# zijinxuxu/PDFNet

Hardware: AMD Instinct MI355X
Metric: train-step images/sec @256x256 RGB-D B=32 (higher is better)
Workload: dtype f32

## Files before the change

include/pdfnet_hip.h:

```cpp
#ifndef PDFNET_HIP_H
#define PDFNET_HIP_H
#ifdef __cplusplus
extern "C" {
#endif

#define PDF_E_BADARG (-1)
#define PDF_E_WORKSPACE (-2)
#define PDF_ACT_NONE 0
#define PDF_ACT_RELU 1
#define PDF_ACT_LRELU01 2


int pdf_linear_fwd(const float* x, const float* w, const float* bias, float* y,
                   int M, int N, int K, int ldx, int ldw, int ldy, int act, void* stream);
int pdf_linear_bwd_weight(const float* x, const float* dy, float* dw, float* db, float* ws, long ws_floats,
                          int M, int N, int K, int ldx, int lddy, int accumulate, void* stream);
long pdf_wgrad_workspace_floats(int M, int NI, int NJ);
int pdf_init(void);
int pdf_debug_init_device(void);
int pdf_debug_kernel_timing(int on);
int pdf_set_stats_output(float* part, long cap_floats);
long pdf_stats_result_tiles(void);
long pdf_stats_result_rows(void);
int pdf_set_bn_tile_stats(const float* part, long tiles, long rows_per_tile);
// ... 230 lines not shown
int pdf_mano_split_coeff_bwd(const float* params, float* dparams, int ldp, long HW, const long* ind, const float* K, int B, int input_res, int down,
                             const float* dorient, const float* dpose, const float* dtrans, void* stream);


typedef struct PdfCallOpts {
    const void* op0_bf16; const void* op1_bf16;
    void* out_bf16;
    const void* bn_x_bf16;
    float* stats_out; long stats_cap;
    long stats_tiles; long stats_rows;
    const float* tile_stats; long tile_n; long tile_rows;
    const float* in_scale; const float* in_shift;
    const void* op1_bf16_t;
    float* ws; long ws_floats;
    const float* wino_v;
} PdfCallOpts;
long pdf_conv2d_winograd_v_offset(int N, int H, int W, int Cin, int Cout, int KH, int KW, int stride, int pad);
int pdf_linear_fwd_x(const float* x, const float* w, const float* bias, float* y, int M, int N, int K, int ldx, int ldw, int ldy, int act, void* stream, PdfCallOpts* opts);
int pdf_linear_fwd_pair_x(const float* x, const float* w0, const float* w1, const float* b0, const float* b1, float* y, int M, int N, int K, int ldx, int ldw, int ldy, int act, void* stream, PdfCallOpts* opts);
int pdf_linear_bwd_data_x(const float* dy, const float* w, float* dx, int M, int N, int K, int lddy, int ldw, int lddx, void* stream, PdfCallOpts* opts);
int pdf_linear_bwd_data_pair_x(const float* dy, const float* w0, const float* w1, float* dx, int M, int N, int K, int lddy, int ldw, int lddx, void* stream, PdfCallOpts* opts);
int pdf_conv2d_fwd_x(const float* x, const float* w, const float* bias, float* y, int N, int H, int W, int Cin, int ldx, int Cout, int KH, int KW, int stride, int pad, int OH, int OW, int ldy, int act, void* stream, PdfCallOpts* opts);
int pdf_conv2d_bwd_data_x(const float* dy, const float* w, float* dx, int N, int H, int W, int Cin, int lddx, int Cout, int KH, int KW, int stride, int pad, int OH, int OW, int lddy, void* stream, PdfCallOpts* opts);
int pdf_conv2d_bwd_data_add_x(const float* dy, const float* w, float* dx, int N, int H, int W, int Cin, int lddx, int Cout, int KH, int KW, int stride, int pad, int OH, int OW, int lddy, void* stream, PdfCallOpts* opts);
int pdf_linear_bwd_weight_x(const float* x, const float* dy, float* dw, float* db, float* ws, long ws_floats, int M, int N, int K, int ldx, int lddy, int accumulate, void* stream, PdfCallOpts* opts);
int pdf_linear_bwd_weight_pair_x(const float* x, const float* dy, float* dw0, float* dw1, float* db0, float* db1, float* ws, long ws_floats, int M, int N, int K, int ldx, int lddy, int accumulate, void* stream, PdfCallOpts* opts);
int pdf_conv2d_bwd_weight_x(const float* x, const float* dy, float* dw, float* db, float* ws, long ws_floats, int N, int H, int W, int Cin, int ldx, int Cout, int KH, int KW, int stride, int pad, int OH, int OW, int lddy, int accumulate, void* stream, PdfCallOpts* opts);
int pdf_deconv2d_fwd_x(const float* x, const float* w, const float* bias, float* y, int N, int H, int W, int Cin, int ldx, int Cout, int KH, int KW, int stride, int pad, int OH, int OW, int ldy, void* stream, PdfCallOpts* opts);
int pdf_deconv2d_bwd_data_x(const float* dy, const float* w, float* dx, int N, int H, int W, int Cin, int lddx, int Cout, int KH, int KW, int stride, int pad, int OH, int OW, int lddy, void* stream, PdfCallOpts* opts);
int pdf_deconv2d_bwd_weight_x(const float* x, const float* dy, float* dw, float* ws, long ws_floats, int N, int H, int W, int Cin, int ldx, int Cout, int KH, int KW, int stride, int pad, int OH, int OW, int lddy, int accumulate, void* stream, PdfCallOpts* opts);
int pdf_bn_train_fwd_x(const float* x, int ldx, int C, long R, const float* gamma, const float* beta, float* running_mean, float* running_var, float momentum, float eps, const float* res, int ldr, int relu, float* y, int ldy, float* save_mean, float* save_rstd, float* scale, float* shift, float* ws, void* stream, PdfCallOpts* opts);
int pdf_bn_train_bwd_x(const float* dy, int lddy, const float* y, int ldy, int relu, const float* x, int ldx, const float* save_mean, const float* save_rstd, const float* gamma, const float* scale, const float* shift, int C, long R, float* dx, int lddx, float* dres, int lddr, float* dgamma, float* dbeta, int accumulate, float* ws, void* stream, PdfCallOpts* opts);
int pdf_bn_relu_maxk_fwd_x(const float* y, int ldy, int C, long R, int K, const float* gamma, const float* beta, float* running_mean, float* running_var, float momentum, float eps, int training, float* out, int ldo, int* arg, float* save_mean, float* save_rstd, float* scale, float* shift, float* ws, void* stream, PdfCallOpts* opts);
int pdf_l2norm_cat_fwd_x(int nparts, const float* const* x, const int* C, const float* const* w, float eps, long R, float* y, int ldy, float* const* norm, void* stream, PdfCallOpts* opts);
long pdf_conv2d_winograd_workspace_floats(int N, int H, int W, int Cin, int Cout, int KH, int KW, int stride, int pad, int backward);
int pdf_debug_armed_slots(void);
int pdf_debug_callopts_size(void);

int pdf_x3_split(const float* x, void* out, long n, long cs, void* stream);
long pdf_deconv2d_x3_workspace_floats(int N, int H, int W, int Cin, int Cout, int KH, int KW, int stride, int pad, int backward);
int pdf_set_x3_mode(int mode);
int pdf_stream_create(void** out, int priority, int* lo, int* hi);
int pdf_debug_x3_mode(void);
int pdf_debug_x3_stamps(unsigned long long* out);
int pdf_x3_batched_gemm_nt(const void* A3, long csA, const void* B3, long csB, float* C, int batch, long gsA, long gsB, long gsC, int M, int N, int K, int variant, int nprod, void* stream);
int pdf_batched_gemm_nt(const float* A, const float* B, float* C, int batch, long gsA, long gsB, long gsC, int M, int N, int K, void* stream);
int pdf_x3_batched_gemm_tn(const void* P3, long csP, const void* Q3, long csQ, float* slab, int batch, long gsP, long gsQ, int M, int NI, int NJ, int splits, int variant, int nprod, void* stream);
int pdf_batched_gemm_tn(const float* P, const float* Q, float* slab, int batch, long gsP, long gsQ, int M, int NI, int NJ, int splits, void* stream);

typedef struct PdfMeshLin { const float* w[2]; const float* b[2]; } PdfMeshLin;
typedef struct PdfMeshLN { const float* g[2]; const float* b[2]; } PdfMeshLN;
typedef struct PdfMeshGcn { PdfMeshLin fc1, fc2, sc; PdfMeshLN n2, n3; unsigned long long seed; } PdfMeshGcn;
typedef struct PdfMeshAttn {
    PdfMeshLN ln; PdfMeshLin q, k, v, fc; PdfMeshLN ffln; PdfMeshLin f1, f2;
    unsigned long long seed_att, seed_z, seed_t, seed_x;
// ... 55 lines not shown
```

pdfnet_amd/csrc/gemm.hip:

```cpp
#include "common.h"

#include "gemm_common.h"
#include "gemm_internal.h"

PDF_API long pdf_conv2d_winograd_v_offset(int N, int H, int W, int Cin, int Cout, int KH, int KW, int stride, int pad) {
    if (!pdf_internal_wino_eligible(N, H, W, Cin, Cout, KH, KW, stride, pad, 0) || !pdf_internal_wino_wgrad_eligible(N, H, W, Cin, Cout, KH, KW, stride, pad)) return -1;
    return pdf_internal_wino_v_offset(N, H, W, Cin, Cout);
}
PDF_API long pdf_conv2d_winograd_workspace_floats(int N, int H, int W, int Cin, int Cout, int KH, int KW, int stride, int pad, int backward) {
    if (backward == 2) return pdf_internal_wino_wgrad_eligible(N, H, W, Cin, Cout, KH, KW, stride, pad) ? pdf_internal_wino_wgrad_workspace(N, H, W, Cin, Cout) : 0;
    const int Ck = backward ? Cout : Cin, Cn = backward ? Cin : Cout;
    return pdf_internal_wino_eligible(N, H, W, Ck, Cn, KH, KW, stride, pad, backward) ? pdf_internal_wino_workspace(N, H, W, Ck, Cn, backward) : 0;
}

constexpr int WG_ISSUE_AT = 1;
typedef unsigned int u32x4v __attribute__((ext_vector_type(4)));
__device__ __forceinline__ float4 as_f4(const u32x4v& v) { return *reinterpret_cast<const float4*>(&v); }

template <int BM, int BN, int WM, int WN, bool FAST, bool KN, int BKT, bool BUF, bool AFF>
__device__ __forceinline__ void igemm_nt_body(const IGemm& g) {
    constexpr int NT = WM * WN * 64;
    constexpr int BK = BKT, LD = BK + 1;
    constexpr int TM = BM / WM / 32, TN = BN / WN / 32;
    constexpr int TPR = BK / 4, RPP = NT / TPR;
// ... 1319 lines not shown
}

int pdf_internal_batched_gemm(const float* A, const float* B, float* C, int batch, long gsA, long gsB, long gsC, int M, int N, int K, hipStream_t s) {
    IGemm g = {};
    g.A = A; g.B = B; g.C = C; g.bias = nullptr;
    g.M = M; g.N = N; g.K = K; g.Cin = K; g.lda = K; g.ldb = K; g.ldc = N;
    g.T = 1; g.plain_in = 1; g.plain_out = 1; g.act = 0;
    g.H = 1; g.W = M; g.QH = 1; g.QW = M; g.sy = 1; g.sx = 1;
    g.batch = batch; g.gsA = gsA; g.gsB = gsB; g.gsC = gsC;
    if (g_gemm_bf16) return PDF_E_BADARG;
    return launch_igemm(g, s, batch);
}

PDF_API long pdf_deconv2d_x3_workspace_floats(int N, int H, int W, int Cin, int Cout, int KH, int KW, int stride, int pad, int backward) {
    return g_gemm_bf16 ? 0 : pdf_internal_x3_deconv_workspace(N, H, W, Cin, Cout, KH, KW, stride, pad, backward);
}
static void conv_taps(IGemm& g, int KH, int KW, int pad, int dil) {
    g.T = KH * KW;
    for (int ky = 0; ky < KH; ++ky)
        for (int kx = 0; kx < KW; ++kx) {
            int t = ky * KW + kx;
            g.dy[t] = (int)(ky * dil - pad); g.dx[t] = (int)(kx * dil - pad); g.wt[t] = t;
        }
}

static IGemm linear_desc(const float* x, const float* w, const float* bias, float* y,
                         int M, int N, int K, int ldx, int ldw, int ldy, int act) {
    IGemm g = {};
    g.A = x; g.B = w; g.C = y; g.bias = bias;
    g.M = M; g.N = N; g.K = K; g.Cin = K; g.lda = ldx; g.ldb = ldw; g.ldc = ldy;
// ... 820 lines not shown
PDF_API int pdf_deconv2d_bwd_data(const float* dy, const float* w, float* dx,
                                  int N, int H, int W, int Cin, int lddx, int Cout, int KH, int KW,
                                  int stride, int pad, int OH, int OW, int lddy, void* stream) {
    return pdf_call_plain(pdf_deconv2d_bwd_data_impl, dy, w, dx, N, H, W, Cin, lddx, Cout, KH, KW, stride, pad, OH, OW, lddy, stream);
}


static int pdf_deconv2d_bwd_weight_impl(const float* x, const float* dy, float* dw, float* ws, long ws_floats,
                                    int N, int H, int W, int Cin, int ldx, int Cout, int KH, int KW,
                                    int stride, int pad, int OH, int OW, int lddy, int accumulate, void* stream, PdfCallOpts& co) {
    hipStream_t s = (hipStream_t)stream;
    if (KH * KW > MAX_TAPS) return PDF_E_BADARG;
    if (!g_gemm_bf16 && co.ws != nullptr && ldx == Cin && lddy == Cout) {
        const long need = pdf_internal_x3_deconv_workspace(N, H, W, Cin, Cout, KH, KW, stride, pad, 2);
        if (need > 0 && co.ws_floats >= need && ((uintptr_t)co.ws & 15) == 0) {
            if (KH != stride || pad != 0) return pdf_internal_x3_deconv_general_bwd_weight(x, dy, dw, co.ws, N, H, W, Cin, Cout, KH, stride, pad, OH, OW, lddy, accumulate, s);
            return pdf_internal_x3_deconv_bwd_weight(x, dy, dw, co.ws, N, H, W, Cin, Cout, KH, KW, stride, OH, OW, lddy, accumulate, s);
        }
    }
    WGemm g = {};
    g.P = x; g.Q = dy; g.P16 = co.op0_bf16; g.Q16 = co.op1_bf16; g.M = N * H * W; g.NI = Cin; g.Cq = Cout; g.T = KH * KW;
    g.ldp = ldx; g.ldq = lddy; g.ldw = KH * KW * Cout;
    g.H = OH; g.W = OW; g.QH = H; g.QW = W; g.sy = stride; g.sx = stride; g.plain_q = 0;
    for (int ky = 0; ky < KH; ++ky)
        for (int kx = 0; kx < KW; ++kx) {
            int t = ky * KW + kx;
            g.dy[t] = (int)(ky - pad); g.dx[t] = (int)(kx - pad); g.wt[t] = t;
        }
    return launch_wgemm(g, dw, ws, ws_floats, accumulate, s);
}
PDF_API int pdf_deconv2d_bwd_weight_x(const float* x, const float* dy, float* dw, float* ws, long ws_floats,
                                    int N, int H, int W, int Cin, int ldx, int Cout, int KH, int KW,
                                    int stride, int pad, int OH, int OW, int lddy, int accumulate, void* stream, PdfCallOpts* opts) {
    return pdf_call_x(opts, pdf_deconv2d_bwd_weight_impl, x, dy, dw, ws, ws_floats, N, H, W, Cin, ldx, Cout, KH, KW, stride, pad, OH, OW, lddy,
// ... 10 lines not shown
```

pdfnet_amd/csrc/gemm_internal.h:

```cpp
#pragma once
#include "common.h"

int pdf_internal_batched_gemm(const float* A, const float* B, float* C, int batch, long gsA, long gsB, long gsC, int M, int N, int K, hipStream_t s);
int pdf_internal_batched_wgemm(const float* P, const float* Q, float* slab, int batch, long gsP, long gsQ, int M, int NI, int NJ, int splits, hipStream_t s);

long pdf_internal_wino_workspace(int N, int H, int W, int Ck, int Cn, int flip);
int pdf_internal_wino_eligible(int N, int H, int W, int Ck, int Cn, int KH, int KW, int stride, int pad, int flip);
int pdf_internal_conv3x3_winograd(const float* x, int ldx, const float* w, const float* bias, float* y, int ldy, float* ws,
                                  int N, int H, int W, int Ck, int Cn, int act, int accum, int flip, const float* v_shared, hipStream_t s);
int pdf_internal_wino_wgrad_eligible(int N, int H, int W, int Cin, int Cout, int KH, int KW, int stride, int pad);
long pdf_internal_wino_wgrad_workspace(int N, int H, int W, int Cin, int Cout);
long pdf_internal_wino_v_offset(int N, int H, int W, int Ck, int Cn);
int pdf_internal_conv3x3_winograd_wgrad(const float* x, int ldx, const float* dy, int lddy, float* dw, float* db, float* ws,
                                        int N, int H, int W, int Cin, int Cout, int accumulate, const float* v_cached, hipStream_t s);

int pdf_internal_x3_mode();
int pdf_internal_x3_batched_gemm(const void* A3, long csA, const void* B3, long csB, float* C, int batch, long gsA, long gsB, long gsC,
                                 int M, int N, int K, int variant, int nprod, hipStream_t s);
int pdf_internal_x3_batched_wgemm(const void* P3, long csP, const void* Q3, long csQ, float* slab, int batch, long gsP, long gsQ,
                                  int M, int NI, int NJ, int splits, int variant, int nprod, hipStream_t s);
long pdf_internal_x3_deconv_workspace(int N, int H, int W, int Cin, int Cout, int KH, int KW, int stride, int pad, int backward);
int pdf_internal_x3_deconv_fwd(const float* x, const float* w, const float* bias, float* y, float* ws, int N, int H, int W, int Cin, int Cout,
                               int KH, int KW, int stride, int OH, int OW, int ldy, hipStream_t s);
int pdf_internal_x3_deconv_bwd_data(const float* dy, const float* w, float* dx, float* ws, int N, int H, int W, int Cin, int lddx, int Cout,
                                    int KH, int KW, int stride, int OH, int OW, int lddy, hipStream_t s);
int pdf_internal_x3_deconv_general_fwd(const float* x, const float* w, const float* bias, float* y, float* ws, int N, int H, int W, int Cin, int Cout,
                                       int K, int stride, int pad, int OH, int OW, int ldy, hipStream_t s);
int pdf_internal_x3_deconv_general_bwd_data(const float* dy, const float* w, float* dx, float* ws, int N, int H, int W, int Cin, int lddx, int Cout,
                                            int K, int stride, int pad, int OH, int OW, int lddy, hipStream_t s);
int pdf_internal_x3_deconv_general_bwd_weight(const float* x, const float* dy, float* dw, float* ws, int N, int H, int W, int Cin, int Cout,
                                              int K, int stride, int pad, int OH, int OW, int lddy, int accumulate, hipStream_t s);
int pdf_internal_x3_deconv_bwd_weight(const float* x, const float* dy, float* dw, float* ws, int N, int H, int W, int Cin, int Cout,
                                      int KH, int KW, int stride, int OH, int OW, int lddy, int accumulate, hipStream_t s);
```

pdfnet_amd/csrc/gemm_x3.hip:

```cpp
#include "gemm_common.h"
#include "gemm_internal.h"
#include <cstdio>

typedef __bf16 bf16x8v __attribute__((ext_vector_type(8)));
typedef short s16x4v __attribute__((ext_vector_type(4)));
typedef short s16x8v __attribute__((ext_vector_type(8)));
typedef int i32x4 __attribute__((ext_vector_type(4)));

__device__ __forceinline__ i32x4 x3_rsrc(const void* p, unsigned bytes) {
    const unsigned long long a = (unsigned long long)p;
    i32x4 r = {(int)(unsigned)(a & 0xffffffffu), (int)(unsigned)((a >> 32) & 0xffffu), (int)bytes, 0x00020000};
    return r;
}
__device__ __forceinline__ void x3_dma16(const i32x4& rsrc, unsigned lds_addr, unsigned voff) {
    asm volatile("s_mov_b32 m0, %0\n\tbuffer_load_dwordx4 %1, %2, 0 offen lds" ::"s"(lds_addr), "v"(voff), "s"(rsrc) : "memory");
}

__global__ __launch_bounds__(256) void x3_split_kernel(const float* __restrict__ x, unsigned short* __restrict__ o, long n8, long cs) {
    for (long i = blockIdx.x * 256L + threadIdx.x; i < n8; i += (long)gridDim.x * 256) {
        const float4 u = reinterpret_cast<const float4*>(x)[2 * i], v = reinterpret_cast<const float4*>(x)[2 * i + 1];
        uint4 h, m, l;
        pdf_x3_split2(u.x, u.y, h.x, m.x, l.x); pdf_x3_split2(u.z, u.w, h.y, m.y, l.y);
        pdf_x3_split2(v.x, v.y, h.z, m.z, l.z); pdf_x3_split2(v.z, v.w, h.w, m.w, l.w);
        *reinterpret_cast<uint4*>(o + 8 * i) = h;
// ... 679 lines not shown
PDF_API int pdf_set_x3_mode(int mode) { g_x3_mode = mode < 0 ? -1 : (mode & 7); return 0; }
PDF_API int pdf_debug_x3_mode(void) { return pdf_internal_x3_mode(); }
static int x3_deconv_mode() { return (pdf_internal_x3_mode() & 2) != 0; }
static long x3_ld(long K) { return K + 64; }
static long x3_deconv_general_workspace(int N, int H, int W, int Cin, int Cout, int K, int stride, int pad, int backward);
long pdf_internal_x3_deconv_workspace(int N, int H, int W, int Cin, int Cout, int KH, int KW, int stride, int pad, int backward) {
    if (!x3_deconv_mode() || KH != KW || stride < 2) return 0;
    if (KH != stride || pad != 0) return x3_deconv_general_workspace(N, H, W, Cin, Cout, KH, stride, pad, backward);
    const long M = (long)N * H * W, NT = (long)KH * KW * Cout;
    if (Cin % 32 != 0 || Cout % 32 != 0 || M < 1024 || 2.0 * M * NT * Cin < 3.0e10) return 0;
    if (backward == 2 && (M % 32 != 0 || 3.0 * Cin * NT * 4.0 >= 4294967000.0)) return 0;
    const long wel = backward == 2 ? M * x3_ld(Cin) : backward ? Cin * x3_ld(NT) : NT * x3_ld(Cin), ael = backward ? M * x3_ld(NT) : M * x3_ld(Cin);
    if (3.0 * wel >= 2147483000.0 || 3.0 * ael >= 2147483000.0) return 0;
    return ((3 * wel + 1) / 2 + 3) / 4 * 4 + ((3 * ael + 1) / 2 + 3) / 4 * 4 + 64;
}
static void x3_gemm_desc(X3Gemm& g, const void* A3, long csA, long lda, const void* B3, long csB, long ldb, float* C, int M, int N, int K, int ldc) {
    g = X3Gemm{};
    g.A = (const unsigned short*)A3; g.B = (const unsigned short*)B3; g.C = C;
    g.csA = csA; g.csB = csB; g.M = M; g.N = N; g.K = K; g.batch = 1; g.ldc = ldc; g.lda = (int)lda; g.ldb = (int)ldb;
    g.col_major_tiles = cdiv(N, 128) > 4 * cdiv(M, 128);
}
static int x3_launch_auto(const X3Gemm& g, hipStream_t s) {
    const int v = x3_nt_variant(g.M, g.N, g.K, g.batch);
    if (v == 0) return x3_launch_nt<4, 2, 2, 2, 2>(g, 6, s);
    if (v == 1) return x3_launch_nt<2, 2, 2, 2, 3>(g, 6, s);
    return x3_launch_nt<2, 4, 2, 1, 3>(g, 6, s);
}
int pdf_internal_x3_deconv_fwd(const float* x, const float* w, const float* bias, float* y, float* ws, int N, int H, int W, int Cin, int Cout,
                               int KH, int KW, int stride, int OH, int OW, int ldy, hipStream_t s) {
    const long M = (long)N * H * W, NT = (long)KH * KW * Cout, ld = x3_ld(Cin);
    unsigned short* w3 = reinterpret_cast<unsigned short*>(ws);
    unsigned short* x3 = reinterpret_cast<unsigned short*>(ws + ((3 * NT * ld + 1) / 2 + 3) / 4 * 4);
    {
        KTimer kt("x3_split_transpose_kernel", 0.0, 10.0 * NT * Cin, s);
        hipLaunchKernelGGL(x3_split_transpose_kernel, dim3((unsigned)cdiv(NT, 64), (unsigned)cdiv(Cin, 64)), dim3(256), 0, s, w, NT, w3, Cin, (int)NT, ld, NT * ld, X3TrJobs{});
    }
    hipLaunchKernelGGL(x3_split_rows_kernel, dim3(grid_for(M * Cin / 8, 256, 256 * 16)), dim3(256), 0, s, x, (long)Cin, x3, ld, M * ld, M, Cin / 8);
    PDF_LAUNCH_CHECK();
    X3Gemm g;
    x3_gemm_desc(g, x3, M * ld, ld, w3, NT * ld, ld, y, (int)M, (int)NT, Cin, ldy);
    g.ps_cout = Cout; g.ps_kw = KW; g.ps_s = stride; g.QH = H; g.QW = W; g.OH = OH; g.OW = OW; g.bias = bias;
    return x3_launch_auto(g, s);
}
int pdf_internal_x3_deconv_bwd_data(const float* dy, const float* w, float* dx, float* ws, int N, int H, int W, int Cin, int lddx, int Cout,
                                    int KH, int KW, int stride, int OH, int OW, int lddy, hipStream_t s) {
    const long M = (long)N * H * W, NT = (long)KH * KW * Cout, ld = x3_ld(NT);
    unsigned short* w3 = reinterpret_cast<unsigned short*>(ws);
    unsigned short* d3 = reinterpret_cast<unsigned short*>(ws + ((3 * Cin * ld + 1) / 2 + 3) / 4 * 4);
    {
        KTimer kt("x3_split_rows_kernel", 0.0, 10.0 * NT * Cin, s);
        hipLaunchKernelGGL(x3_split_rows_kernel, dim3(grid_for(NT * Cin / 8, 256, 256 * 16)), dim3(256), 0, s, w, NT, w3, ld, Cin * ld, (long)Cin, (int)(NT / 8));
    }
    {
        KTimer kt("x3_split_unshuffle_kernel", 0.0, 10.0 * M * NT, s);
        hipLaunchKernelGGL(x3_split_unshuffle_kernel, dim3(grid_for(M * NT / 8, 256, 256 * 16)), dim3(256), 0, s, dy, lddy, d3, ld, M * ld, M, H, W, OH, OW, stride, Cout);
    }
    PDF_LAUNCH_CHECK();
    X3Gemm g;
    x3_gemm_desc(g, d3, M * ld, ld, w3, Cin * ld, ld, dx, (int)M, Cin, (int)NT, lddx);
    return x3_launch_auto(g, s);
}

int pdf_internal_x3_deconv_bwd_weight(const float* x, const float* dy, float* dw, float* ws, int N, int H, int W, int Cin, int Cout,
                                      int KH, int KW, int stride, int OH, int OW, int lddy, int accumulate, hipStream_t s) {
    const long M = (long)N * H * W, NT = (long)KH * KW * Cout, ldx3 = x3_ld(Cin), ldd = x3_ld(NT);
    unsigned short* x3 = reinterpret_cast<unsigned short*>(ws);
    unsigned short* d3 = reinterpret_cast<unsigned short*>(ws + ((3 * M * ldx3 + 1) / 2 + 3) / 4 * 4);
    hipLaunchKernelGGL(x3_split_rows_kernel, dim3(grid_for(M * Cin / 8, 256, 256 * 16)), dim3(256), 0, s, x, (long)Cin, x3, ldx3, M * ldx3, M, Cin / 8);
    {
        KTimer kt("x3_split_unshuffle_kernel", 0.0, 10.0 * M * NT, s);
        hipLaunchKernelGGL(x3_split_unshuffle_kernel, dim3(grid_for(M * NT / 8, 256, 256 * 16)), dim3(256), 0, s, dy, lddy, d3, ldd, M * ldd, M, H, W, OH, OW, stride, Cout);
    }
    PDF_LAUNCH_CHECK();
    X3Gemm g = {};
    g.A = x3; g.B = d3; g.C = dw;
    g.csA = M * ldx3; g.csB = M * ldd; g.lda = (int)ldx3; g.ldb = (int)ldd;
    g.M = Cin; g.N = (int)NT; g.K = (int)M; g.batch = 1; g.splits = 1; g.rows_per_split = (int)M; g.accum = accumulate;
    return x3_launch_tn_deconv(g, s);
}

static bool x3_general_ok(int Cin, int Cout, int K, int stride, int pad) {
    return K % stride == 0 && K * K <= 16 && K > stride && pad >= 0 && pad < K && Cin % 32 == 0 && Cout % 32 == 0;
}
static int x3_general_wgrad_splits(long M, int NI, long NJ) {
    const long tiles = (long)cdiv(NI, 128) * cdiv(NJ, 128);
    long sp = (512 + tiles - 1) / tiles;
// ... 43 lines not shown
                    const int pc = py * stride + px;
                    tky[pc][n] = ky; tkx[pc][n] = kx;
                    jobs.in_off[pc * T + n] = (long)(ky * K + kx) * Cout;
                    jobs.out_off[pc * T + n] = (long)pc * Cout * ldB + (long)n * Cin;
                    ++n;
                }
            }
            if (n != T) return PDF_E_BADARG;
        }
    {
        KTimer kt("x3_split_transpose_kernel", 0.0, 10.0 * K * K * Cout * Cin, s);
        hipLaunchKernelGGL(x3_split_transpose_kernel, dim3((unsigned)cdiv(Cout, 64), (unsigned)cdiv(Cin, 64), (unsigned)(P * T)), dim3(256), 0, s,
                           w, (long)K * K * Cout, b3, Cin, Cout, ldB, (long)P * Cout * ldB, jobs);
    }
    hipLaunchKernelGGL(x3_split_rows_kernel, dim3(grid_for(Min * Cin / 8, 256, 256 * 16)), dim3(256), 0, s, x, (long)Cin, a3, ldA, (Min + 1) * ldA, Min, Cin / 8);
    if (int rc = x3_zero_rows(a3, Min, ldA, s)) return rc;
    PDF_LAUNCH_CHECK();
    for (int py = 0; py < stride; ++py)
        for (int px = 0; px < stride; ++px) {
            const int pc = py * stride + px, QH = (OH - py + stride - 1) / stride, QW = (OW - px + stride - 1) / stride;
            X3Gemm g;
            x3_gemm_desc(g, a3, (Min + 1) * ldA, ldA, b3 + (long)pc * Cout * ldB, (long)P * Cout * ldB, ldB, y, N * QH * QW, Cout, T * Cin, ldy);
            g.ps_cout = Cout; g.ps_kw = 1; g.ps_s = stride; g.QH = QH; g.QW = QW; g.OH = OH; g.OW = OW; g.ooy = py; g.oox = px; g.bias = bias;
            g.AH = H; g.AW = W; g.sy = 1; g.sx = 1; g.T = T; g.Cc = Cin; g.zrow = Min * ldA;
            for (int n = 0; n < T; ++n) {
                g.tdy[n] = (py + pad - tky[pc][n]) / stride; g.tdx[n] = (px + pad - tkx[pc][n]) / stride;
            }
            if (int rc = x3_launch_auto(g, s)) return rc;
        }
    return 0;
}
int pdf_internal_x3_deconv_general_bwd_data(const float* dy, const float* w, float* dx, float* ws, int N, int H, int W, int Cin, int lddx, int Cout,
                                            int K, int stride, int pad, int OH, int OW, int lddy, hipStream_t s) {
    const long Mout = (long)N * OH * OW, M = (long)N * H * W, NT = (long)K * K * Cout;
    const long ldA = x3_ld(Cout), ldB = x3_ld(NT);
    unsigned short* b3 = reinterpret_cast<unsigned short*>(ws);
    unsigned short* a3 = reinterpret_cast<unsigned short*>(ws + ((3 * Cin * ldB + 1) / 2 + 3) / 4 * 4);
    {
        KTimer kt("x3_split_rows_kernel", 0.0, 10.0 * NT * Cin, s);
        hipLaunchKernelGGL(x3_split_rows_kernel, dim3(grid_for(NT * Cin / 8, 256, 256 * 16)), dim3(256), 0, s, w, NT, b3, ldB, Cin * ldB, (long)Cin, (int)(NT / 8));
    }
    {
        KTimer kt("x3_split_rows_kernel", 0.0, 10.0 * Mout * Cout, s);
        hipLaunchKernelGGL(x3_split_rows_kernel, dim3(grid_for(Mout * Cout / 8, 256, 256 * 16)), dim3(256), 0, s, dy, (long)lddy, a3, ldA, (Mout + 1) * ldA, Mout, Cout / 8);
    }
    if (int rc = x3_zero_rows(a3, Mout, ldA, s)) return rc;
    PDF_LAUNCH_CHECK();
    X3Gemm g;
    x3_gemm_desc(g, a3, (Mout + 1) * ldA, ldA, b3, Cin * ldB, ldB, dx, (int)M, Cin, (int)NT, lddx);
    g.QH = H; g.QW = W; g.AH = OH; g.AW = OW; g.sy = stride; g.sx = stride; g.T = K * K; g.Cc = Cout; g.zrow = Mout * ldA;
    for (int ky = 0; ky < K; ++ky)
        for (int kx = 0; kx < K; ++kx) { g.tdy[ky * K + kx] = ky - pad; g.tdx[ky * K + kx] = kx - pad; }
    return x3_launch_auto(g, s);
}

__global__ __launch_bounds__(256) void x3_slab_reduce_kernel(const float* __restrict__ slab, int splits, long n4, float* __restrict__ dw, int accumulate) {
    for (long i = blockIdx.x * 256L + threadIdx.x; i < n4; i += (long)gridDim.x * 256) {
        float4 v = reinterpret_cast<const float4*>(slab)[i];
        for (int y = 1; y < splits; ++y) { const float4 u = reinterpret_cast<const float4*>(slab)[(long)y * n4 + i]; v.x += u.x; v.y += u.y; v.z += u.z; v.w += u.w; }
        if (accumulate) { const float4 u = reinterpret_cast<const float4*>(dw)[i]; v.x += u.x; v.y += u.y; v.z += u.z; v.w += u.w; }
        reinterpret_cast<float4*>(dw)[i] = v;
    }
}
int pdf_internal_x3_deconv_general_bwd_weight(const float* x, const float* dy, float* dw, float* ws, int N, int H, int W, int Cin, int Cout,
                                              int K, int stride, int pad, int OH, int OW, int lddy, int accumulate, hipStream_t s) {
    const long Min = (long)N * H * W, Mout = (long)N * OH * OW, NT = (long)K * K * Cout;
    const long ldP = x3_ld(Cin), ldQ = x3_ld(Cout);
    unsigned short* p3 = reinterpret_cast<unsigned short*>(ws);
    float* wq = ws + ((3 * Min * ldP + 1) / 2 + 3) / 4 * 4;
    unsigned short* q3 = reinterpret_cast<unsigned short*>(wq);
    float* slab = wq + ((3 * (Mout + 1) * ldQ + 1) / 2 + 3) / 4 * 4;
    hipLaunchKernelGGL(x3_split_rows_kernel, dim3(grid_for(Min * Cin / 8, 256, 256 * 16)), dim3(256), 0, s, x, (long)Cin, p3, ldP, Min * ldP, Min, Cin / 8);
    {
        KTimer kt("x3_split_rows_kernel", 0.0, 10.0 * Mout * Cout, s);
        hipLaunchKernelGGL(x3_split_rows_kernel, dim3(grid_for(Mout * Cout / 8, 256, 256 * 16)), dim3(256), 0, s, dy, (long)lddy, q3, ldQ, (Mout + 1) * ldQ, Mout, Cout / 8);
    }
    if (int rc = x3_zero_rows(q3, Mout, ldQ, s)) return rc;
    PDF_LAUNCH_CHECK();
    const int splits = x3_general_wgrad_splits(Min, Cin, NT);
    X3Gemm g = {};
    g.A = p3; g.B = q3; g.C = splits > 1 ? slab : dw;
    g.csA = Min * ldP; g.csB = (Mout + 1) * ldQ; g.lda = (int)ldP; g.ldb = (int)ldQ;
    g.M = Cin; g.N = (int)NT; g.K = (int)Min; g.batch = 1;
    g.rows_per_split = cdiv(cdiv(Min, splits), 32) * 32; g.splits = cdiv(Min, g.rows_per_split);
    g.accum = (g.splits == 1) ? accumulate : 0;
    g.QH = H; g.QW = W; g.AH = OH; g.AW = OW; g.sy = stride; g.sx = stride; g.T = K * K; g.Cc = Cout; g.zrow = Mout * ldQ;
    g.lw = __builtin_ctz(W); g.lhw = __builtin_ctz(H * W);
    for (int ky = 0; ky < K; ++ky)
        for (int kx = 0; kx < K; ++kx) { g.tdy[ky * K + kx] = ky - pad; g.tdx[ky * K + kx] = kx - pad; }
    if (g.splits == 1) g.C = dw;
    if (int rc = x3_launch_tn_deconv(g, s)) return rc;
    if (g.splits > 1) {
        KTimer kt("x3_slab_reduce_kernel", 0.0, 4.0 * (g.splits + 1) * Cin * NT, s);
        hipLaunchKernelGGL(x3_slab_reduce_kernel, dim3(grid_for((long)Cin * NT / 4)), dim3(256), 0, s, slab, g.splits, (long)Cin * NT / 4, dw, accumulate);
        PDF_LAUNCH_CHECK();
    }
    return 0;
// ... 2 lines not shown
```

pdfnet_amd/functional.py:

```python
import ctypes
import torch
from torch.autograd import Function

from . import hip
from .hip import ptr, ptr_at, stream

ACT_NONE, ACT_RELU, ACT_LRELU = 0, 1, 2
import os as _os

_byref = ctypes.byref
_CallOpts = hip.CallOpts
USE_SIDE_STREAMS = _os.environ.get("PDFNET_SIDE_STREAMS", "1") != "0"
_side = {}


def _record(obj, stream_):
    if torch.is_tensor(obj):
        obj.record_stream(stream_)
        s16 = getattr(obj, '_pdf_bf16', None)
        if s16 is not None:
            s16.record_stream(stream_)
    elif isinstance(obj, (list, tuple)):
        for o in obj:
            _record(o, stream_)
# ... 166 lines not shown
        n = _wino_cache[key] = _L().pdf_conv2d_winograd_workspace_floats(N, H, W, Cin, Cout, KH, KW, stride, pad, backward)
    if n <= 0:
        return None, None
    return torch.empty(n, dtype=torch.float32, device=dev), n


X3_DECONV = _os.environ.get("PDFNET_X3_DECONV", "1") != "0"
_x3d_cache = {}


def set_x3(mode):
    _L().pdf_set_x3_mode(-1 if mode is None else int(mode))
    _wino_cache.clear()
    _wino_voff.clear()
    _x3d_cache.clear()


def _x3_deconv_ws(N, H, W, Cin, Cout, KH, KW, stride, pad, backward, dev):
    if not X3_DECONV or _GEMM_BF16 or KH != KW or stride < 2:
        return None, None
    key = (N, H, W, Cin, Cout, KH, stride, pad, backward)
    n = _x3d_cache.get(key)
    if n is None:
        n = _x3d_cache[key] = _L().pdf_deconv2d_x3_workspace_floats(N, H, W, Cin, Cout, KH, KW, stride, pad, backward)
    if n <= 0:
        return None, None
    return torch.empty(n, dtype=torch.float32, device=dev), n


WINOGRAD_KEEP_V = _os.environ.get("PDFNET_WINOGRAD_KEEP_V", "1") != "0"
_wino_voff = {}


def _wino_v_offset(N, H, W, Cin, Cout, KH, KW, stride, pad):
    key = (N, H, W, Cin, Cout, KH, KW, stride, pad)
    off = _wino_voff.get(key)
    if off is None:
        off = _wino_voff[key] = _L().pdf_conv2d_winograd_v_offset(N, H, W, Cin, Cout, KH, KW, stride, pad)
    return off


WINOGRAD_SHARE = _os.environ.get("PDFNET_WINOGRAD_SHARE", "1") != "0"
# ... 381 lines not shown
    @staticmethod
    def forward(ctx, x, w, b, stride, pad):
        hip.require_gpu(x, w)
        w_in = w
        x, w = cl(x), cl(w)
        N, Cin, H, W = x.shape
        _, Cout, KH, KW = w.shape
        OH = (H - 1) * stride - 2 * pad + KH
        OW = (W - 1) * stride - 2 * pad + KW
        L = _L()
        y = torch.empty((N, Cout, OH, OW), dtype=torch.float32, device=x.device, memory_format=CL)
        x16, w16 = shadow_of(x), shadow_of(w)
        ws, nws = _x3_deconv_ws(N, H, W, Cin, Cout, KH, KW, stride, pad, 0, x.device)
        L.pdf_deconv2d_fwd_x(ptr(x), ptr(w), ptr(b), ptr(y), N, H, W, Cin, Cin, Cout, KH, KW, stride, pad, OH, OW, Cout, stream(),
                             _O(op0_bf16=ptr(x16), op1_bf16=ptr(w16), ws=ptr(ws), ws_floats=nws)[1])
        ctx.save_for_backward(x, w)
        ctx.s16 = (x16, w16)
        ctx.cfg = (stride, pad, b is not None)
        ctx.params = (w_in, b)
        return y

    @staticmethod
    def backward(ctx, dy):
        x, w = ctx.saved_tensors
        stride, pad, has_b = ctx.cfg
        N, Cin, H, W = x.shape
        _, Cout, KH, KW = w.shape
        OH, OW = dy.shape[2], dy.shape[3]
        g = cl(dy)
        x16, w16 = ctx.s16
        g16 = shadow_of(g)
        L = _L()
        dx = dw = db = None
        if ctx.needs_input_grad[0]:
            dx = torch.empty_like(x)
            ws, nws = _x3_deconv_ws(N, H, W, Cin, Cout, KH, KW, stride, pad, 1, x.device)
            L.pdf_deconv2d_bwd_data_x(ptr(g), ptr(w), ptr(dx), N, H, W, Cin, Cin, Cout, KH, KW, stride, pad, OH, OW, Cout, stream(),
                                      _O(op0_bf16=ptr(g16), op1_bf16=ptr(w16), ws=ptr(ws), ws_floats=nws)[1])
        w_par, b_par = ctx.params

        def launch_w(out, out_b, acc):
            ws, n = _wgrad_ws(N * H * W, Cin, KH * KW * Cout, x.device)
            xws, nx = _x3_deconv_ws(N, H, W, Cin, Cout, KH, KW, stride, pad, 2, x.device)
            L.pdf_deconv2d_bwd_weight_x(ptr(x), ptr(g), ptr(out), ptr(ws), n, N, H, W, Cin, Cin, Cout, KH, KW,
                                        stride, pad, OH, OW, Cout, acc, stream(), _O(op0_bf16=ptr(x16), op1_bf16=ptr(g16), ws=ptr(xws), ws_floats=nx)[1])
        dw, db = _param_grads(ctx, x, g, w, w_par, b_par, has_b, launch_w, Cout, N * OH * OW, 2.0 * N * H * W * Cin * KH * KW * Cout, shadows=(x16, g16))
        return dx, dw, db, None, None


def deconv2d(x, w, b=None, stride=1, pad=0):
    return _Deconv2d.apply(x, w, b, stride, pad)


class _Linear(Function):

    @staticmethod
    def forward(ctx, x, w, b, act, fp32=False, stats=False):
        hip.require_gpu(x, w)
        w_in = w
        lz = _lazy_bn(x)
        if lz is not None:
# ... 2062 lines not shown
```

pdfnet_amd/taped.py:

```python
import os

import torch
from torch.autograd import Function
from torch.utils._python_dispatch import TorchDispatchMode

from . import functional as F
from . import hip

TRUNK_TAPE = os.environ.get("PDFNET_TRUNK_TAPE", "1") != "0"
SUSPEND = False

SWITCHES = ('WINOGRAD', 'WINOGRAD_KEEP_V', 'WINOGRAD_SHARE', 'BN_EPILOGUE_STATS', 'BN_EPILOGUE_STATS_BF16', 'ASYNC_WGRAD_MIN_FLOP',
            'BF16_SHADOWS', 'TRANSPOSED_SHADOWS')

_ALLOC = ('empty', 'empty_like', 'empty_strided', 'new_empty', 'record_stream')
_VIEW = ('view', 'reshape', '_unsafe_view', 'permute', 'transpose', 'expand', 'slice', 'select', 'squeeze', 'unsqueeze', 't.', 'alias', 'detach',
         'as_strided', 'unbind', 'split', 'contiguous', '_reshape_alias', 'narrow', 'flatten', 'unflatten')


class _Recorder(TorchDispatchMode):

    def __init__(self, tape, pins):
        super().__init__()
        self.tape, self.pins, self.refused = tape, pins, []

    def __torch_dispatch__(self, func, types, args=(), kwargs=None):
        out = func(*args, **(kwargs or {}))
        name = str(func).replace('aten.', '')
# ... 224 lines not shown
```

Before: 728.8.

## Reuse x3-split activation planes from deconv forward/bwd-data in weight gradient

Measured after the change: 732.3, median of 6. About the same (+0.5%).

```diff
diff --git a/include/pdfnet_hip.h b/include/pdfnet_hip.h
--- a/include/pdfnet_hip.h
+++ b/include/pdfnet_hip.h
@@ -268,6 +268,8 @@
     const void* op1_bf16_t;
     float* ws; long ws_floats;
     const float* wino_v;
+    const void* x3_x; long x3_x_tag;
+    const void* x3_dy; long x3_dy_tag;
 } PdfCallOpts;
 long pdf_conv2d_winograd_v_offset(int N, int H, int W, int Cin, int Cout, int KH, int KW, int stride, int pad);
 int pdf_linear_fwd_x(const float* x, const float* w, const float* bias, float* y, int M, int N, int K, int ldx, int ldw, int ldy, int act, void* stream, PdfCallOpts* opts);
@@ -293,6 +295,8 @@
 
 int pdf_x3_split(const float* x, void* out, long n, long cs, void* stream);
 long pdf_deconv2d_x3_workspace_floats(int N, int H, int W, int Cin, int Cout, int KH, int KW, int stride, int pad, int backward);
+long pdf_deconv2d_x3_planes(int N, int H, int W, int Cin, int Cout, int KH, int KW, int stride, int pad, int pass, long* tag);
+long pdf_debug_x3_act_splits(int which, int reset);
 int pdf_set_x3_mode(int mode);
 int pdf_stream_create(void** out, int priority, int* lo, int* hi);
 int pdf_debug_x3_mode(void);
diff --git a/pdfnet_amd/csrc/gemm.hip b/pdfnet_amd/csrc/gemm.hip
--- a/pdfnet_amd/csrc/gemm.hip
+++ b/pdfnet_amd/csrc/gemm.hip
@@ -1357,6 +1357,10 @@
 
 PDF_API long pdf_deconv2d_x3_workspace_floats(int N, int H, int W, int Cin, int Cout, int KH, int KW, int stride, int pad, int backward) {
     return g_gemm_bf16 ? 0 : pdf_internal_x3_deconv_workspace(N, H, W, Cin, Cout, KH, KW, stride, pad, backward);
+}
+PDF_API long pdf_deconv2d_x3_planes(int N, int H, int W, int Cin, int Cout, int KH, int KW, int stride, int pad, int pass, long* tag) {
+    if (tag) *tag = 0;
+    return g_gemm_bf16 ? -1 : pdf_internal_x3_deconv_planes(N, H, W, Cin, Cout, KH, KW, stride, pad, pass, tag);
 }
 static void conv_taps(IGemm& g, int KH, int KW, int pad, int dil) {
     g.T = KH * KW;
@@ -2207,10 +2211,12 @@
     if (!g_gemm_bf16 && co.ws != nullptr && ldx == Cin && lddy == Cout) {
         const long need = pdf_internal_x3_deconv_workspace(N, H, W, Cin, Cout, KH, KW, stride, pad, 2);
         if (need > 0 && co.ws_floats >= need && ((uintptr_t)co.ws & 15) == 0) {
-            if (KH != stride || pad != 0) return pdf_internal_x3_deconv_general_bwd_weight(x, dy, dw, co.ws, N, H, W, Cin, Cout, KH, stride, pad, OH, OW, lddy, accumulate, s);
-            return pdf_internal_x3_deconv_bwd_weight(x, dy, dw, co.ws, N, H, W, Cin, Cout, KH, KW, stride, OH, OW, lddy, accumulate, s);
-        }
-    }
+            if (KH != stride || pad != 0) return pdf_internal_x3_deconv_general_bwd_weight(x, dy, dw, co.ws, N, H, W, Cin, Cout, KH, stride, pad, OH, OW, lddy, accumulate,
+                                                                                           co.x3_x, co.x3_x_tag, co.x3_dy, co.x3_dy_tag, s);
+            return pdf_internal_x3_deconv_bwd_weight(x, dy, dw, co.ws, N, H, W, Cin, Cout, KH, KW, stride, OH, OW, lddy, accumulate, co.x3_x, co.x3_x_tag, co.x3_dy, co.x3_dy_tag, s);
+        }
+    }
+    if (co.x3_x != nullptr || co.x3_dy != nullptr) return PDF_E_BADARG;
     WGemm g = {};
     g.P = x; g.Q = dy; g.P16 = co.op0_bf16; g.Q16 = co.op1_bf16; g.M = N * H * W; g.NI = Cin; g.Cq = Cout; g.T = KH * KW;
     g.ldp = ldx; g.ldq = lddy; g.ldw = KH * KW * Cout;
diff --git a/pdfnet_amd/csrc/gemm_internal.h b/pdfnet_amd/csrc/gemm_internal.h
--- a/pdfnet_amd/csrc/gemm_internal.h
+++ b/pdfnet_amd/csrc/gemm_internal.h
@@ -29,6 +29,9 @@
 int pdf_internal_x3_deconv_general_bwd_data(const float* dy, const float* w, float* dx, float* ws, int N, int H, int W, int Cin, int lddx, int Cout,
                                             int K, int stride, int pad, int OH, int OW, int lddy, hipStream_t s);
 int pdf_internal_x3_deconv_general_bwd_weight(const float* x, const float* dy, float* dw, float* ws, int N, int H, int W, int Cin, int Cout,
-                                              int K, int stride, int pad, int OH, int OW, int lddy, int accumulate, hipStream_t s);
+                                              int K, int stride, int pad, int OH, int OW, int lddy, int accumulate,
+                                              const void* x_planes, long x_tag, const void* dy_planes, long dy_tag, hipStream_t s);
 int pdf_internal_x3_deconv_bwd_weight(const float* x, const float* dy, float* dw, float* ws, int N, int H, int W, int Cin, int Cout,
-                                      int KH, int KW, int stride, int OH, int OW, int lddy, int accumulate, hipStream_t s);
+                                      int KH, int KW, int stride, int OH, int OW, int lddy, int accumulate,
+                                      const void* x_planes, long x_tag, const void* dy_planes, long dy_tag, hipStream_t s);
+long pdf_internal_x3_deconv_planes(int N, int H, int W, int Cin, int Cout, int KH, int KW, int stride, int pad, int pass, long* tag);
diff --git a/pdfnet_amd/csrc/gemm_x3.hip b/pdfnet_amd/csrc/gemm_x3.hip
--- a/pdfnet_amd/csrc/gemm_x3.hip
+++ b/pdfnet_amd/csrc/gemm_x3.hip
@@ -717,6 +717,47 @@
     if (3.0 * wel >= 2147483000.0 || 3.0 * ael >= 2147483000.0) return 0;
     return ((3 * wel + 1) / 2 + 3) / 4 * 4 + ((3 * ael + 1) / 2 + 3) / 4 * 4 + 64;
 }
+static long x3_ws_floats(long el) { return ((el + 1) / 2 + 3) / 4 * 4; }
+static long x3_act_tag(int kind, long rows, long ld, int zrow, int stride) {
+    if (rows >= (1L << 28) || ld >= (1L << 24) || stride >= 128) return 0;
+    return ((long)kind << 60) | ((long)zrow << 59) | ((long)stride << 52) | (ld << 28) | rows;
+}
+static void x3_deconv_wgrad_tags(int N, int H, int W, int Cin, int Cout, int KH, int KW, int stride, int pad, long* tx, long* td) {
+    *tx = *td = 0;
+    if (pdf_internal_x3_deconv_workspace(N, H, W, Cin, Cout, KH, KW, stride, pad, 2) <= 0) return;
+    const long M = (long)N * H * W;
+    if (KH != stride || pad != 0) {
+        *tx = x3_act_tag(1, M, x3_ld(Cin), 1, 0);
+    } else {
+        *tx = x3_act_tag(1, M, x3_ld(Cin), 0, 0);
+        *td = x3_act_tag(2, M, x3_ld((long)KH * KW * Cout), 0, stride);
+    }
+}
+long pdf_internal_x3_deconv_planes(int N, int H, int W, int Cin, int Cout, int KH, int KW, int stride, int pad, int pass, long* tag) {
+    if (tag) *tag = 0;
+    if (pass != 0 && pass != 1) return -1;
+    if (pdf_internal_x3_deconv_workspace(N, H, W, Cin, Cout, KH, KW, stride, pad, pass) <= 0) return -1;
+    long tx, td;
+    x3_deconv_wgrad_tags(N, H, W, Cin, Cout, KH, KW, stride, pad, &tx, &td);
+    const long t = pass ? td : tx;
+    if (t == 0) return -1;
+    const long NT = (long)KH * KW * Cout;
+    long off;
+    if (KH != stride || pad != 0) {
+        const long kk = KH / stride;
+        off = pass ? x3_ws_floats(3 * Cin * x3_ld(NT)) : x3_ws_floats(3 * (long)stride * stride * Cout * x3_ld(kk * kk * Cin));
+    } else {
+        off = pass ? x3_ws_floats(3 * Cin * x3_ld(NT)) : x3_ws_floats(3 * NT * x3_ld(Cin));
+    }
+    if (tag) *tag = t;
+    return off;
+}
+static long g_x3_act_splits[2];
+static void x3_count_split(int which) { __atomic_fetch_add(&g_x3_act_splits[which], 1L, __ATOMIC_RELAXED); }
+PDF_API long pdf_debug_x3_act_splits(int which, int reset) {
+    if (which < 0 || which > 1) return PDF_E_BADARG;
+    return reset ? __atomic_exchange_n(&g_x3_act_splits[which], 0L, __ATOMIC_RELAXED) : __atomic_load_n(&g_x3_act_splits[which], __ATOMIC_RELAXED);
+}
 static void x3_gemm_desc(X3Gemm& g, const void* A3, long csA, long lda, const void* B3, long csB, long ldb, float* C, int M, int N, int K, int ldc) {
     g = X3Gemm{};
     g.A = (const unsigned short*)A3; g.B = (const unsigned short*)B3; g.C = C;
@@ -739,6 +780,7 @@
         hipLaunchKernelGGL(x3_split_transpose_kernel, dim3((unsigned)cdiv(NT, 64), (unsigned)cdiv(Cin, 64)), dim3(256), 0, s, w, NT, w3, Cin, (int)NT, ld, NT * ld, X3TrJobs{});
     }
     hipLaunchKernelGGL(x3_split_rows_kernel, dim3(grid_for(M * Cin / 8, 256, 256 * 16)), dim3(256), 0, s, x, (long)Cin, x3, ld, M * ld, M, Cin / 8);
+    x3_count_split(0);
     PDF_LAUNCH_CHECK();
     X3Gemm g;
     x3_gemm_desc(g, x3, M * ld, ld, w3, NT * ld, ld, y, (int)M, (int)NT, Cin, ldy);
@@ -757,6 +799,7 @@
     {
         KTimer kt("x3_split_unshuffle_kernel", 0.0, 10.0 * M * NT, s);
         hipLaunchKernelGGL(x3_split_unshuffle_kernel, dim3(grid_for(M * NT / 8, 256, 256 * 16)), dim3(256), 0, s, dy, lddy, d3, ld, M * ld, M, H, W, OH, OW, stride, Cout);
+        x3_count_split(1);
     }
     PDF_LAUNCH_CHECK();
     X3Gemm g;
@@ -765,14 +808,26 @@
 }
 
 int pdf_internal_x3_deconv_bwd_weight(const float* x, const float* dy, float* dw, float* ws, int N, int H, int W, int Cin, int Cout,
-                                      int KH, int KW, int stride, int OH, int OW, int lddy, int accumulate, hipStream_t s) {
+                                      int KH, int KW, int stride, int OH, int OW, int lddy, int accumulate,
+                                      const void* x_planes, long x_tag, const void* dy_planes, long dy_tag, hipStream_t s) {
     const long M = (long)N * H * W, NT = (long)KH * KW * Cout, ldx3 = x3_ld(Cin), ldd = x3_ld(NT);
-    unsigned short* x3 = reinterpret_cast<unsigned short*>(ws);
-    unsigned short* d3 = reinterpret_cast<unsigned short*>(ws + ((3 * M * ldx3 + 1) / 2 + 3) / 4 * 4);
-    hipLaunchKernelGGL(x3_split_rows_kernel, dim3(grid_for(M * Cin / 8, 256, 256 * 16)), dim3(256), 0, s, x, (long)Cin, x3, ldx3, M * ldx3, M, Cin / 8);
-    {
+    long tx, td;
+    x3_deconv_wgrad_tags(N, H, W, Cin, Cout, KH, KW, stride, 0, &tx, &td);
+    if ((x_planes && (x_tag != tx || tx == 0 || ((uintptr_t)x_planes & 15))) || (dy_planes && (dy_tag != td || td == 0 || ((uintptr_t)dy_planes & 15)))) return PDF_E_BADARG;
+    const unsigned short* x3 = reinterpret_cast<const unsigned short*>(x_planes);
+    const unsigned short* d3 = reinterpret_cast<const unsigned short*>(dy_planes);
+    if (!x3) {
+        unsigned short* o = reinterpret_cast<unsigned short*>(ws);
+        hipLaunchKernelGGL(x3_split_rows_kernel, dim3(grid_for(M * Cin / 8, 256, 256 * 16)), dim3(256), 0, s, x, (long)Cin, o, ldx3, M * ldx3, M, Cin / 8);
+        x3_count_split(0);
+        x3 = o;
+    }
+    if (!d3) {
+        unsigned short* o = reinterpret_cast<unsigned short*>(ws + ((3 * M * ldx3 + 1) / 2 + 3) / 4 * 4);
         KTimer kt("x3_split_unshuffle_kernel", 0.0, 10.0 * M * NT, s);
-        hipLaunchKernelGGL(x3_split_unshuffle_kernel, dim3(grid_for(M * NT / 8, 256, 256 * 16)), dim3(256), 0, s, dy, lddy, d3, ldd, M * ldd, M, H, W, OH, OW, stride, Cout);
+        hipLaunchKernelGGL(x3_split_unshuffle_kernel, dim3(grid_for(M * NT / 8, 256, 256 * 16)), dim3(256), 0, s, dy, lddy, o, ldd, M * ldd, M, H, W, OH, OW, stride, Cout);
+        x3_count_split(1);
+        d3 = o;
     }
     PDF_LAUNCH_CHECK();
     X3Gemm g = {};
@@ -846,6 +901,7 @@
                            w, (long)K * K * Cout, b3, Cin, Cout, ldB, (long)P * Cout * ldB, jobs);
     }
     hipLaunchKernelGGL(x3_split_rows_kernel, dim3(grid_for(Min * Cin / 8, 256, 256 * 16)), dim3(256), 0, s, x, (long)Cin, a3, ldA, (Min + 1) * ldA, Min, Cin / 8);
+    x3_count_split(0);
     if (int rc = x3_zero_rows(a3, Min, ldA, s)) return rc;
     PDF_LAUNCH_CHECK();
     for (int py = 0; py < stride; ++py)
@@ -875,6 +931,7 @@
     {
         KTimer kt("x3_split_rows_kernel", 0.0, 10.0 * Mout * Cout, s);
         hipLaunchKernelGGL(x3_split_rows_kernel, dim3(grid_for(Mout * Cout / 8, 256, 256 * 16)), dim3(256), 0, s, dy, (long)lddy, a3, ldA, (Mout + 1) * ldA, Mout, Cout / 8);
+        x3_count_split(1);
     }
     if (int rc = x3_zero_rows(a3, Mout, ldA, s)) return rc;
     PDF_LAUNCH_CHECK();
@@ -895,24 +952,36 @@
     }
 }
 int pdf_internal_x3_deconv_general_bwd_weight(const float* x, const float* dy, float* dw, float* ws, int N, int H, int W, int Cin, int Cout,
-                                              int K, int stride, int pad, int OH, int OW, int lddy, int accumulate, hipStream_t s) {
+                                              int K, int stride, int pad, int OH, int OW, int lddy, int accumulate,
+                                              const void* x_planes, long x_tag, const void* dy_planes, long dy_tag, hipStream_t s) {
     const long Min = (long)N * H * W, Mout = (long)N * OH * OW, NT = (long)K * K * Cout;
     const long ldP = x3_ld(Cin), ldQ = x3_ld(Cout);
-    unsigned short* p3 = reinterpret_cast<unsigned short*>(ws);
+    long tx, td;
+    x3_deconv_wgrad_tags(N, H, W, Cin, Cout, K, K, stride, pad, &tx, &td);
+    if ((x_planes && (x_tag != tx || tx == 0 || ((uintptr_t)x_planes & 15))) || (dy_planes && (dy_tag != td || td == 0 || ((uintptr_t)dy_planes & 15)))) return PDF_E_BADARG;
     float* wq = ws + ((3 * Min * ldP + 1) / 2 + 3) / 4 * 4;
+    float* slab = wq + ((3 * (Mout + 1) * ldQ + 1) / 2 + 3) / 4 * 4;
+    const unsigned short* p3 = reinterpret_cast<const unsigned short*>(x_planes);
     unsigned short* q3 = reinterpret_cast<unsigned short*>(wq);
-    float* slab = wq + ((3 * (Mout + 1) * ldQ + 1) / 2 + 3) / 4 * 4;
-    hipLaunchKernelGGL(x3_split_rows_kernel, dim3(grid_for(Min * Cin / 8, 256, 256 * 16)), dim3(256), 0, s, x, (long)Cin, p3, ldP, Min * ldP, Min, Cin / 8);
+    long csP = (Min + 1) * ldP;
+    if (!p3) {
+        unsigned short* o = reinterpret_cast<unsigned short*>(ws);
+        csP = Min * ldP;
+        hipLaunchKernelGGL(x3_split_rows_kernel, dim3(grid_for(Min * Cin / 8, 256, 256 * 16)), dim3(256), 0, s, x, (long)Cin, o, ldP, csP, Min, Cin / 8);
+        x3_count_split(0);
+        p3 = o;
+    }
     {
         KTimer kt("x3_split_rows_kernel", 0.0, 10.0 * Mout * Cout, s);
         hipLaunchKernelGGL(x3_split_rows_kernel, dim3(grid_for(Mout * Cout / 8, 256, 256 * 16)), dim3(256), 0, s, dy, (long)lddy, q3, ldQ, (Mout + 1) * ldQ, Mout, Cout / 8);
+        x3_count_split(1);
     }
     if (int rc = x3_zero_rows(q3, Mout, ldQ, s)) return rc;
     PDF_LAUNCH_CHECK();
     const int splits = x3_general_wgrad_splits(Min, Cin, NT);
     X3Gemm g = {};
     g.A = p3; g.B = q3; g.C = splits > 1 ? slab : dw;
-    g.csA = Min * ldP; g.csB = (Mout + 1) * ldQ; g.lda = (int)ldP; g.ldb = (int)ldQ;
+    g.csA = csP; g.csB = (Mout + 1) * ldQ; g.lda = (int)ldP; g.ldb = (int)ldQ;
     g.M = Cin; g.N = (int)NT; g.K = (int)Min; g.batch = 1;
     g.rows_per_split = cdiv(cdiv(Min, splits), 32) * 32; g.splits = cdiv(Min, g.rows_per_split);
     g.accum = (g.splits == 1) ? accumulate : 0;
diff --git a/pdfnet_amd/functional.py b/pdfnet_amd/functional.py
--- a/pdfnet_amd/functional.py
+++ b/pdfnet_amd/functional.py
@@ -204,6 +204,7 @@
     _wino_cache.clear()
     _wino_voff.clear()
     _x3d_cache.clear()
+    _x3p_cache.clear()
 
 
 def _x3_deconv_ws(N, H, W, Cin, Cout, KH, KW, stride, pad, backward, dev):
@@ -216,6 +217,23 @@
     if n <= 0:
         return None, None
     return torch.empty(n, dtype=torch.float32, device=dev), n
+
+
+PREPARED_OPERANDS = _os.environ.get("PDFNET_PREPARED_OPERANDS", "1") != "0"
+_x3p_cache = {}
+
+
+def _x3_deconv_planes(N, H, W, Cin, Cout, KH, KW, stride, pad, which):
+    if not PREPARED_OPERANDS or not X3_DECONV or _GEMM_BF16 or KH != KW or stride < 2:
+        return None
+    key = (N, H, W, Cin, Cout, KH, stride, pad, which)
+    ent = _x3p_cache.get(key)
+    if ent is None:
+        import ctypes as _ct
+        tag = _ct.c_long(0)
+        off = _L().pdf_deconv2d_x3_planes(N, H, W, Cin, Cout, KH, KW, stride, pad, which, _ct.byref(tag))
+        ent = _x3p_cache[key] = (off, tag.value)
+    return ent if ent[0] >= 0 else None
 
 
 WINOGRAD_KEEP_V = _os.environ.get("PDFNET_WINOGRAD_KEEP_V", "1") != "0"
@@ -627,6 +645,11 @@
         ws, nws = _x3_deconv_ws(N, H, W, Cin, Cout, KH, KW, stride, pad, 0, x.device)
         L.pdf_deconv2d_fwd_x(ptr(x), ptr(w), ptr(b), ptr(y), N, H, W, Cin, Cin, Cout, KH, KW, stride, pad, OH, OW, Cout, stream(),
                              _O(op0_bf16=ptr(x16), op1_bf16=ptr(w16), ws=ptr(ws), ws_floats=nws)[1])
+        ctx.x3_x = None
+        if ws is not None and ctx.needs_input_grad[1]:
+            pl = _x3_deconv_planes(N, H, W, Cin, Cout, KH, KW, stride, pad, 0)
+            if pl is not None:
+                ctx.x3_x = (ws, pl[0], pl[1])
         ctx.save_for_backward(x, w)
         ctx.s16 = (x16, w16)
         ctx.cfg = (stride, pad, b is not None)
@@ -645,19 +668,35 @@
         g16 = shadow_of(g)
         L = _L()
         dx = dw = db = None
+        keep_x, keep_g = ctx.x3_x, None
+        ctx.x3_x = None
         if ctx.needs_input_grad[0]:
             dx = torch.empty_like(x)
             ws, nws = _x3_deconv_ws(N, H, W, Cin, Cout, KH, KW, stride, pad, 1, x.device)
             L.pdf_deconv2d_bwd_data_x(ptr(g), ptr(w), ptr(dx), N, H, W, Cin, Cin, Cout, KH, KW, stride, pad, OH, OW, Cout, stream(),
                                       _O(op0_bf16=ptr(g16), op1_bf16=ptr(w16), ws=ptr(ws), ws_floats=nws)[1])
+            if ws is not None and ctx.needs_input_grad[1]:
+                pl = _x3_deconv_planes(N, H, W, Cin, Cout, KH, KW, stride, pad, 1)
+                if pl is not None:
+                    keep_g = (ws, pl[0], pl[1])
         w_par, b_par = ctx.params
 
         def launch_w(out, out_b, acc):
             ws, n = _wgrad_ws(N * H * W, Cin, KH * KW * Cout, x.device)
             xws, nx = _x3_deconv_ws(N, H, W, Cin, Cout, KH, KW, stride, pad, 2, x.device)
+            px = pg = None
+            if xws is not None:
+                if keep_x is not None and _x3_deconv_planes(N, H, W, Cin, Cout, KH, KW, stride, pad, 0) == keep_x[1:]:
+                    px = keep_x
+                if keep_g is not None and _x3_deconv_planes(N, H, W, Cin, Cout, KH, KW, stride, pad, 1) == keep_g[1:]:
+                    pg = keep_g
             L.pdf_deconv2d_bwd_weight_x(ptr(x), ptr(g), ptr(out), ptr(ws), n, N, H, W, Cin, Cin, Cout, KH, KW,
-                                        stride, pad, OH, OW, Cout, acc, stream(), _O(op0_bf16=ptr(x16), op1_bf16=ptr(g16), ws=ptr(xws), ws_floats=nx)[1])
-        dw, db = _param_grads(ctx, x, g, w, w_par, b_par, has_b, launch_w, Cout, N * OH * OW, 2.0 * N * H * W * Cin * KH * KW * Cout, shadows=(x16, g16))
+                                        stride, pad, OH, OW, Cout, acc, stream(),
+                                        _O(op0_bf16=ptr(x16), op1_bf16=ptr(g16), ws=ptr(xws), ws_floats=nx,
+                                           x3_x=(px[0].data_ptr() + 4 * px[1]) if px is not None else None, x3_x_tag=px[2] if px is not None else None,
+                                           x3_dy=(pg[0].data_ptr() + 4 * pg[1]) if pg is not None else None, x3_dy_tag=pg[2] if pg is not None else None)[1])
+        dw, db = _param_grads(ctx, x, g, w, w_par, b_par, has_b, launch_w, Cout, N * OH * OW, 2.0 * N * H * W * Cin * KH * KW * Cout,
+                              shadows=(x16, g16, keep_x[0] if keep_x is not None else None, keep_g[0] if keep_g is not None else None))
         return dx, dw, db, None, None
 
 
diff --git a/pdfnet_amd/taped.py b/pdfnet_amd/taped.py
--- a/pdfnet_amd/taped.py
+++ b/pdfnet_amd/taped.py
@@ -11,7 +11,7 @@
 SUSPEND = False
 
 SWITCHES = ('WINOGRAD', 'WINOGRAD_KEEP_V', 'WINOGRAD_SHARE', 'BN_EPILOGUE_STATS', 'BN_EPILOGUE_STATS_BF16', 'ASYNC_WGRAD_MIN_FLOP',
-            'BF16_SHADOWS', 'TRANSPOSED_SHADOWS')
+            'BF16_SHADOWS', 'TRANSPOSED_SHADOWS', 'PREPARED_OPERANDS')
 
 _ALLOC = ('empty', 'empty_like', 'empty_strided', 'new_empty', 'record_stream')
 _VIEW = ('view', 'reshape', '_unsafe_view', 'permute', 'transpose', 'expand', 'slice', 'select', 'squeeze', 'unsqueeze', 't.', 'alias', 'detach',
```
